# gabrielmpp/LagrangianCoherence

Measured on AMD Instinct MI355X. Metric: particle-timesteps/sec (+ FTLE Mcells/sec) at 4096^2 seeds per GPU, higher is better.
Workload: dtype f32

## Files before the change

### include/lcs_hip.h

```cpp
#ifndef LCS_HIP_H
#define LCS_HIP_H

#include <stddef.h>
#include <stdint.h>

#ifdef __cplusplus
extern "C" {
#endif

#define LC_VERSION 104

typedef struct lc_ctx lc_ctx;

enum lc_dtype {
    LC_F32 = 0,
    LC_F64 = 1,
    LC_F64_WIND_F32 = 2,
    LC_F64_WIND_F32_LIN32 = 3
};

enum lc_status {
    LC_OK = 0,
    LC_EINVAL = -1,
    LC_EUNSUPPORTED = -2,
    LC_EHIP = -3,
    LC_ENOMEM = -4,
    LC_ERCCL = -5
};

enum lc_xboundary {
    LC_X_CLAMP_POINT = 0,
    LC_X_CYCLIC = 1,
    LC_X_CLAMP_REFERENCE_OUTER = 2
};

enum lc_tensor_layout {
    LC_LAYOUT_REFERENCE = 0,
    LC_LAYOUT_PHYSICAL = 1
};

int lc_version(void);
const char *lc_last_error(void);
const char *lc_build_id(void);

int lc_ctx_create(int device, lc_ctx **out);
int lc_ctx_destroy(lc_ctx *ctx);
int lc_ctx_set_stream(lc_ctx *ctx, void *hip_stream );
int lc_ctx_use_own_stream(lc_ctx *ctx);
int lc_sync(lc_ctx *ctx);

int lc_ctx_set_lds_tiles(lc_ctx *ctx, int mode);
int lc_ctx_set_sigma_march(lc_ctx *ctx, int on);
typedef int (*lc_flag_allreduce_fn)(void *user, void *flags_dev, size_t count);
int lc_ctx_set_flag_allreduce(lc_ctx *ctx, lc_flag_allreduce_fn fn, void *user);
int lc_ctx_set_level_chunk(lc_ctx *ctx, int levels);
int lc_ctx_get_level_chunk(const lc_ctx *ctx, int *levels_out);
enum lc_f64_fidelity { LC_F64_AUTO = 0, LC_F64_EXACT_ORDER = 1, LC_F64_FAST = 2 };
#define LC_EXACT_ORDER_MAX_SEEDS (1 << 18)
int lc_ctx_set_f64_fidelity(lc_ctx *ctx, int mode);
int lc_ctx_get_f64_fidelity(const lc_ctx *ctx, int *mode_out);
int lc_ctx_set_host_pipeline(lc_ctx *ctx, int on);
int lc_copy_to_device(lc_ctx *ctx, void *dst_dev, const void *src_host, size_t bytes);
int lc_copy_to_host(lc_ctx *ctx, void *dst_host, const void *src_dev, size_t bytes);
int lc_ctx_set_host_cache(lc_ctx *ctx, int on);
int lc_ctx_trim(lc_ctx *ctx);
int lc_ctx_last_host_marks(const lc_ctx *ctx, double *ms4_out);
int lc_ctx_set_xcd_split(lc_ctx *ctx, int split);
const char *lc_ctx_last_advect_kernel(const lc_ctx *ctx);
int lc_ctx_last_advect_launches(const lc_ctx *ctx);
const char *lc_ctx_last_sigma_kernel(const lc_ctx *ctx);
const char *lc_ctx_last_pack_kernel(const lc_ctx *ctx);
const char *lc_ctx_last_tracer_kernel(const lc_ctx *ctx);
#define LC_VERIFY_WORDS 16
int lc_ctx_set_verify(lc_ctx *ctx, int mode);
int lc_ctx_read_verify(lc_ctx *ctx, unsigned *out16, int reset);

int lc_malloc(lc_ctx *ctx, size_t bytes, void **dev_out);
int lc_free(lc_ctx *ctx, void *dev);
int lc_memcpy_h2d(lc_ctx *ctx, void *dev_dst, const void *host_src, size_t bytes);
int lc_memcpy_d2h(lc_ctx *ctx, void *host_dst, const void *dev_src, size_t bytes);

size_t lc_packed_elems(int nt, int ny_f, int nx_f);
int lc_field_pack(lc_ctx *ctx, const void *u_dev, const void *v_dev, int dtype,
                  int nt, int ny_f, int nx_f, int interp_order, void *packed_dev,
                  void *ext_dev );

int lc_field_extrapolate(lc_ctx *ctx, const void *packed_dev, int dtype,
                         int nt, int ny_f, int nx_f, void *ext_dev);

// ... 153 lines not shown
```

### lagrangiancoherence_amd/_capi.py

```python
from __future__ import annotations

import ctypes as C
import os

HERE = os.path.dirname(os.path.abspath(__file__))
LIB_PATH = os.path.join(HERE, "liblcs_hip.so")

LC_VERSION = 104
LC_F32, LC_F64, LC_F64_WIND_F32, LC_F64_WIND_F32_LIN32 = 0, 1, 2, 3
LC_OK, LC_EINVAL, LC_EUNSUPPORTED, LC_EHIP, LC_ENOMEM, LC_ERCCL = 0, -1, -2, -3, -4, -5
LC_LAYOUT_REFERENCE, LC_LAYOUT_PHYSICAL = 0, 1
LC_X_CLAMP_POINT, LC_X_CYCLIC, LC_X_CLAMP_REFERENCE_OUTER = 0, 1, 2
LC_GRID_REGULAR, LC_GRID_GAUSSIAN = 0, 1
LC_F64_AUTO, LC_F64_EXACT_ORDER, LC_F64_FAST = 0, 1, 2
LC_EXACT_ORDER_MAX_SEEDS = 1 << 18

_vp, _i, _d, _sz = C.c_void_p, C.c_int, C.c_double, C.c_size_t

PROTOTYPES = {
    "lc_version": (_i, []),
    "lc_last_error": (C.c_char_p, []),
    "lc_build_id": (C.c_char_p, []),
    "lc_ctx_create": (_i, [_i, C.POINTER(_vp)]),
    "lc_ctx_destroy": (_i, [_vp]),
    "lc_ctx_set_stream": (_i, [_vp, _vp]),
    "lc_ctx_use_own_stream": (_i, [_vp]),
    "lc_sync": (_i, [_vp]),
    "lc_ctx_set_lds_tiles": (_i, [_vp, _i]),
    "lc_ctx_set_sigma_march": (_i, [_vp, _i]),
    "lc_ctx_set_level_chunk": (_i, [_vp, _i]),
    "lc_ctx_get_level_chunk": (_i, [_vp, C.POINTER(_i)]),
    "lc_ctx_set_f64_fidelity": (_i, [_vp, _i]),
    "lc_ctx_get_f64_fidelity": (_i, [_vp, C.POINTER(_i)]),
    "lc_ctx_set_host_pipeline": (_i, [_vp, _i]),
    "lc_ctx_last_host_marks": (_i, [_vp, C.POINTER(C.c_double)]),
    "lc_copy_to_device": (_i, [_vp, _vp, _vp, C.c_size_t]),
    "lc_copy_to_host": (_i, [_vp, _vp, _vp, C.c_size_t]),
    "lc_ctx_set_host_cache": (_i, [_vp, _i]),
    "lc_ctx_trim": (_i, [_vp]),
    "lc_ctx_set_xcd_split": (_i, [_vp, _i]),
    "lc_ctx_set_flag_allreduce": (_i, [_vp, _vp, _vp]),
    "lc_ctx_last_advect_kernel": (C.c_char_p, [_vp]),
    "lc_ctx_last_advect_launches": (_i, [_vp]),
    "lc_ctx_last_sigma_kernel": (C.c_char_p, [_vp]),
    "lc_ctx_last_pack_kernel": (C.c_char_p, [_vp]),
    "lc_ctx_last_tracer_kernel": (C.c_char_p, [_vp]),
    "lc_ctx_set_verify": (_i, [_vp, _i]),
    "lc_ctx_read_verify": (_i, [_vp, C.POINTER(C.c_uint), _i]),
    "lc_malloc": (_i, [_vp, _sz, C.POINTER(_vp)]),
    "lc_free": (_i, [_vp, _vp]),
    "lc_memcpy_h2d": (_i, [_vp, _vp, _vp, _sz]),
    "lc_memcpy_d2h": (_i, [_vp, _vp, _vp, _sz]),
    "lc_packed_elems": (_sz, [_i, _i, _i]),
    "lc_field_pack": (_i, [_vp, _vp, _vp, _i, _i, _i, _i, _i, _vp, _vp]),
    "lc_field_extrapolate": (_i, [_vp, _vp, _i, _i, _i, _i, _vp]),
    "lc_regrid_common_grid": (_i, [_vp, _vp, _i, _i, _i, _i, _vp, _vp, _vp, _i, _vp, _i, _vp]),
    "lc_spectral_truncate": (_i, [_vp, _vp, _i, _i, _i, _i, _i, _i, _vp]),
    "lc_inspect_gridtype": (_i, [_vp, _i, C.POINTER(_i)]),
    "lc_advect": (_i, [_vp, _vp, _vp, _vp, _i, _i, _i, _i, _d, _d, _d, _d, _vp, _i, _vp, _i, _i, _i,
                       _d, _i, _i, _i, _i, _i, _vp, _vp, _vp, _vp]),
    "lc_advect_from": (_i, [_vp, _vp, _vp, _vp, _i, _i, _i, _i, _d, _d, _d, _d, _vp, _i, _vp, _i, _i, _i, _vp, _vp,
                            _d, _i, _i, _i, _i, _i, _vp, _vp, _vp, _vp]),
    "lc_advect_batch": (_i, [_vp, _vp, _vp, _vp, _i, _i, _i, _i, _d, _d, _d, _d, _vp, _i, _vp, _i, _i, _i, _vp, _vp,
                             _d, _i, _i, _i, _i, _i, _i, _i, _vp, _vp, _vp, _vp]),
# ... 107 lines not shown
```

### lagrangiancoherence_amd/csrc/advect.hip

```cpp
#include <type_traits>
#include <vector>

#include "lcs_common.h"
#include "launch_plan.h"

namespace {

constexpr int TILE_W = 8;
constexpr int TILE_H = 32;
constexpr int BLOCK = TILE_W * TILE_H;

template <typename T>
struct AdvectArgs {
    const T *lin;
    const T *img;
    const T *ext;
    const T *u_raw, *v_raw;
    const float *lin32;
    const float *u_raw32, *v_raw32;
    size_t raw_plane;
    int ext_raw;
    int ext_cub;
    size_t level_elems;
    int pitch;
    int ny_f, nx_f;
    T lat_min, lat_span, lon_min, lon_span;
    T sx, sy;
    T y_min, y_max, x_min, x_max;
    const T *seed_lat, *seed_lon;
    int ny, nx;
    int row0, ny_global;
    T dt, half_dt;
    T dtcy, hdtcy;
    int K, order, cyclic, t0, nsteps;
    int wind_f32;
    T *x_out, *y_out, *traj_x, *traj_y;
    const T *x_start, *y_start;
    int n_members, member_t0_stride;
    size_t member_plane;
    int pair_d, pair_l0, pair_n, pair_g, pair_last;
    size_t pair_plane;
    int traj_skip0;
    int traj_pair_ok, out_pair_ok;
    int traj_line_ok;
    int patch_mode;
    int xcd_rows;
    int xcd_split;
    int wg64;
    int ntx, ntiles;
    int xcd_chunk;
    int tile_order;
    int tile_order_two_seed;
    int pole_blocks, pole_lo, pole_hi;
    unsigned *clamp_flag;
    int clamp_stride;
    unsigned *verify;
    int member_dirs;
};

template <typename T>
__device__ __forceinline__ int xcd_tile_id(const AdvectArgs<T> &A) {
    return lcplan::tile_of_block((int)blockIdx.x - A.pole_blocks, A.ntiles, A.ntx, A.xcd_chunk, A.tile_order);
}
template <typename T>
static inline unsigned nmem(const AdvectArgs<T> &A) { return A.n_members > 1 ? (unsigned)A.n_members : 1u; }

template <typename K, typename T, typename... Extra>
static inline const char *launch_kernel(K kernel, int grid, hipStream_t st, const AdvectArgs<T> &A, const char *name, const Extra &...extra) {
    hipLaunchKernelGGL(kernel, dim3(grid, nmem(A)), dim3(BLOCK), 0, st, A, extra...);
    return name;
}

template <typename T>
struct Pair {
    T u, v;
};

template <typename T>
// ... 1385 lines not shown
            A.traj_y[(size_t)(s + 1) * plane + idx] = p.y;
        }
        lvl += A.level_elems;
        elv += A.level_elems;
    }
    if (live) {
        A.x_out[idx] = p.x;
        A.y_out[idx] = p.y;
    }
}


constexpr int SPL = 2;

#ifndef LCS_LDS2_ROWS
#define LCS_LDS2_ROWS 8
#endif
#ifndef LCS_LDS2_COLS
#define LCS_LDS2_COLS 16
#endif
#ifndef LCS_LDS2_PITCH
#define LCS_LDS2_PITCH (LCS_LDS2_COLS + 4)
#endif
struct Lds2Geom {
    static constexpr int COLS = LCS_LDS2_COLS, LANES_PER_ROW = COLS / 2, ROWS_PER_PASS = 64 / LANES_PER_ROW;
    static_assert(LCS_LDS2_ROWS % ROWS_PER_PASS == 0 || LCS_LDS2_ROWS < ROWS_PER_PASS + 1, "tile rows per staging pass");
};

#ifdef LCS_STAMPS
__device__ unsigned long long g_stamps[8];
__device__ unsigned long long g_cause[4];
__device__ unsigned long long g_redo[3][3][3];
__device__ unsigned long long g_hist[2][5];
#define LCS_STAMP(i)                                           \
    {                                                          \
        const long long _t = __builtin_amdgcn_s_memtime();     \
        acc_t[i] += _t - last_t;                               \
        last_t = _t;                                           \
    }
#else
#define LCS_STAMP(i)
#endif

#ifndef LCS_LDS2_NUM_SGPR
#define LCS_LDS2_NUM_SGPR 96
#endif
constexpr int SLAB_PITCH = 36;

#ifndef LCS_LDS2_MINWAVES
#define LCS_LDS2_MINWAVES 1
#endif
#ifndef LCS_LDS2_DPP_NEXT
#define LCS_LDS2_DPP_NEXT 1
#endif
#ifndef LCS_LDS2_DIRECT_LEVELS
#define LCS_LDS2_DIRECT_LEVELS 0
#endif
template <int KFIX, bool CYCLIC, int MODE>
__global__ void __launch_bounds__(BLOCK, LCS_LDS2_MINWAVES) __attribute__((amdgpu_num_sgpr(LCS_LDS2_NUM_SGPR)))
    advect_lds2_kernel(const AdvectArgs<float> A0) {
#pragma clang fp contract(fast)
    const AdvectArgs<float> A = for_member(A0);
    constexpr bool WIDE = MODE == PATCH_WIDE, LINES = MODE == PATCH_LINES, GROUP = MODE == PATCH_PAIR;
    constexpr int NS = SPL;
    constexpr int ORDER = 1;
    constexpr bool DEFER_X = LCS_LDS2_DEFER_X != 0;
    constexpr int DIRECT_LEVELS = DEFER_X ? LCS_LDS2_DIRECT_LEVELS : 0;
    constexpr bool DPP_NEXT = LCS_LDS2_DPP_NEXT != 0 && 16 % Lds2Geom::LANES_PER_ROW == 0;
    const int K = KFIX >= 0 ? KFIX : A.K;
    typedef Lds2Geom G;
    constexpr int LT_COLS = G::COLS, LT_ROWS = LCS_LDS2_ROWS;
    constexpr int LT_PITCH = LCS_LDS2_PITCH;
    constexpr int WIN = 2, WOFF = LC_PAD_LO;
    __shared__ __attribute__((aligned(16))) f4 s_tiles[BLOCK / 64][LT_ROWS * LT_PITCH];
    __shared__ __attribute__((aligned(16))) float s_slab[2][2][LINES ? 16 * SLAB_PITCH : 4];
    if (GROUP ? pole_block_group(A) : pole_block<float, POLE_LIN>(A)) return;
    const int tile_id = xcd_tile_id(A);
    if (tile_id >= A.ntiles) return;
    const int tyi = tile_id / A.ntx, txi = tile_id - tyi * A.ntx;
    const int lane = threadIdx.x & 63, wave = threadIdx.x >> 6;
    const int ix0 = WIDE ? txi * (TILE_W * SPL) + SPL * (lane % TILE_W)
                  : LINES ? txi * (TILE_W * 4) + wave * TILE_W + (lane % TILE_W) : txi * TILE_W + (lane % TILE_W);
    const int iy0 = (WIDE || GROUP) ? tyi * TILE_H + wave * 8 + lane / TILE_W
                  : LINES ? tyi * (8 * SPL) + lane / TILE_W : tyi * (TILE_H * SPL) + wave * (8 * SPL) + lane / TILE_W;
    f4 *tile = s_tiles[wave];

    bool live[NS];
    f2 p[NS], dd[NS], hd[NS];
    size_t idx[NS];
    const size_t plane = (size_t)A.ny * A.nx;
    bool any = false;
    const int cnt = GROUP ? group_count(A) : NS;
#pragma unroll
    for (int q = 0; q < NS; ++q) {
        const int ix = ix0 + (WIDE ? q : 0), iy = iy0 + ((WIDE || GROUP) ? 0 : 8 * q);
        live[q] = ix < A.nx && iy < A.ny && q < cnt;
        if (live[q]) {
            const int grow = A.row0 + iy;
            if (grow < A.order || grow >= A.ny_global - A.order) {
                if (!A.pole_blocks) {
                    if (GROUP)
                        advect_seed<float, 1, false>(group_member(A, q), A.lin, iy, ix);
                    else
                        advect_seed<float, 1, false>(A, A.lin, iy, ix);
                }
                live[q] = false;
            }
// ... 22 lines not shown
                    dx[off + idx[q]] = p[q].x;
                    dy[off + idx[q]] = p[q].y;
                }
        }
    };
    if (A.traj_x && !A.traj_skip0) store_pair(A.traj_x, A.traj_y, 0);
    const bool lines = LINES && A.traj_x && A.traj_line_ok && (txi + 1) * (TILE_W * 4) <= A.nx;
    if (!lines && __ballot(any) == 0ull) return;
    const int sl_row = (wave & 1) * 8 + (lane >> 3), sl_col = (lane & 7) * 4;
    bool sl_ok = false;
    size_t sl_idx = 0;
    if (lines) {
        const int iyr = tyi * (8 * SPL) + sl_row, grow = A.row0 + iyr;
        sl_ok = iyr < A.ny && (A.pole_blocks == 0 || (grow >= A.order && grow < A.ny_global - A.order));
        if (!A.pole_blocks && iyr < A.ny && (grow < A.order || grow >= A.ny_global - A.order)) sl_ok = false;
        sl_idx = (size_t)min(iyr, A.ny - 1) * A.nx + (size_t)txi * (TILE_W * 4) + sl_col;
    }
    float ymax_v = A.y_max;
    asm volatile("" : "+v"(ymax_v));
    const unsigned tile_addr = lds_address(tile);
    unsigned pitch_bytes = (unsigned)LT_PITCH * 16u;
    asm volatile("" : "+s"(pitch_bytes));
    const f2 pmin = {A.lon_min, A.lat_min}, sc = {A.sx, A.sy};
    auto to_index = [&](f2 v) { return (v - pmin) * sc; };
    const float xlo = A.x_min, xhi = A.x_max;
    auto x_needs_care = [&](float x) { return CYCLIC ? !(fabsf(x) < 180.0f) : !((x > xlo) & (x < xhi)); };
    const float *lvl = A.img + (size_t)A.t0 * A.level_elems;
    const float *elv = A.ext + (size_t)A.t0 * A.level_elems;
    const int pad_cols = A.pitch, pad_rows = A.ny_f + LC_PAD;
    const float kpred = 0.5f * (float)(K > 0 ? K - 1 : 0);
    const int st_row = min(lane / G::LANES_PER_ROW, LT_ROWS - 1), st_col = (lane % G::LANES_PER_ROW) * 2;
    const unsigned st_off = ((unsigned)st_row * (unsigned)pad_cols + (unsigned)st_col) * 8u;
    constexpr int NPASS = (LT_ROWS + G::ROWS_PER_PASS - 1) / G::ROWS_PER_PASS;
    const unsigned st_next = st_off + (st_col + 2 < LT_COLS ? 16u : 0u);
    constexpr int CENTRE = (WIDE || GROUP) ? TILE_W / 2 + TILE_W * 4 : TILE_W / 2 + TILE_W * 7;
    f2 dprev = {0.0f, 0.0f};
    const int nlev = GROUP ? lcplan::group_levels(A.nsteps, A.pair_l0, A.pair_n, A.pair_d, cnt) : A.nsteps;
#ifdef LCS_STAMPS
    long long acc_t[5] = {0, 0, 0, 0, 0}, last_t = __builtin_amdgcn_s_memtime();
    unsigned long long acc_n[3] = {0, 0, 0};
    int prev_redos = 0;
#endif
    int direct_left = 0;
    for (int s = 0; s < nlev; ++s) {
        const bool direct = DIRECT_LEVELS > 0 && direct_left > 0;
        if (direct) --direct_left;
#ifdef LCS_STAMPS
        int level_redos = 0;
#endif
        f2 c0[NS];
#pragma unroll
        for (int q = 0; q < NS; ++q) c0[q] = to_index(p[q]);
        bool act[NS];
        f2 keep[NS];
        int qa = 0;
        if (GROUP) {
            int qlo = NS, qhi = 0;
#pragma unroll
            for (int q = 0; q < NS; ++q) {
                act[q] = lcplan::member_steps(q, s, A.pair_l0, A.pair_n, A.pair_d) && q < cnt;
                keep[q] = p[q];
                if (act[q]) {
                    qlo = min(qlo, q);
                    qhi = q;
                }
            }
            qa = min(max(NS / 2, qlo), qhi);
        }
        auto of_anchor = [&](const f2 (&v)[NS]) {
            f2 r = v[0];
#pragma unroll
            for (int q = 1; q < NS; ++q) r = (GROUP && qa == q) ? v[q] : r;
            return r;
        };
        int ox = 0, oy = 0;
        f4 stage[NPASS];
        f2 stage_next[NPASS];
        if (K > 0 && !direct) {
            const f2 ca = dprev * (1.0f + kpred) + of_anchor(c0);
            const int rxm = __builtin_amdgcn_readlane((int)floor_to_uint(ca.x), CENTRE);
            const int rym = __builtin_amdgcn_readlane((int)floor_to_uint(ca.y), CENTRE);
            ox = min(max(rxm + WOFF - (LT_COLS - WIN) / 2, 0), pad_cols - LT_COLS);
            oy = min(max(rym + WOFF - (LT_ROWS - WIN) / 2, 0), pad_rows - LT_ROWS);
            const char *src = (const char *)elv + ((size_t)__umul24((unsigned)oy, (unsigned)pad_cols) + (unsigned)ox) * 8;
#pragma unroll
            for (int r = 0; r < NPASS; ++r) {
                __builtin_memcpy(&stage[r], src + (size_t)(r * G::ROWS_PER_PASS) * pad_cols * 8 + st_off, 16);
                if (!DPP_NEXT) __builtin_memcpy(&stage_next[r], src + (size_t)(r * G::ROWS_PER_PASS) * pad_cols * 8 + st_next, 8);
            }
        }
        LCS_STAMP(0)
        f2 e[NS], pn[NS];
        bool bad[NS], anybad = false;
#pragma unroll
        for (int q = 0; q < NS; ++q) {
            const TapL t = tap_of(c0[q]);
            bad[q] = ((unsigned)t.x0 > (unsigned)(A.nx_f - 2)) | ((unsigned)t.y0 > (unsigned)(A.ny_f - 2));
            e[q] = euler_global<ORDER>(lvl, A, t);
            pn[q] = dd[q] * e[q] + p[q];
            if (!DEFER_X) bad[q] |= x_needs_care(pn[q].x);
            anybad |= bad[q];
        }
        if (anybad) {
#pragma unroll
            for (int q = 0; q < NS; ++q) {
                if (bad[q]) {
                    const TapL t = tap_of(index_coords(A, p[q]));
                    e[q] = euler_global<ORDER>(lvl, A, t);
                    pn[q] = dd[q] * e[q] + p[q];
                    if (!DEFER_X) clamp_position_p(A, pn[q], ymax_v);
                }
            }
        }
        dprev = (of_anchor(pn) - of_anchor(p)) * sc;
#pragma unroll
        for (int q = 0; q < NS; ++q) p[q] = pn[q];
#ifdef LCS_STAMPS
        asm volatile("" : : "v"(p[0].x), "v"(p[1].x));
#endif
        LCS_STAMP(1)
        int lo_x = 0x40000000, lo_y = 0x40000000, lim_x = 0, lim_y = 0;
        unsigned base_addr = tile_addr;
        if (K > 0 && !direct) {
            __builtin_amdgcn_wave_barrier();
#pragma unroll
            for (int r = 0; r < NPASS; ++r) {
                f2 nxt;
                if constexpr (DPP_NEXT) {
                    float nx0, nx1;
                    const float s0 = stage[r].x, s1 = stage[r].y;
                    asm volatile("s_nop 4\n\tv_mov_b32_dpp %0, %2 row_shl:1 row_mask:0xf bank_mask:0xf bound_ctrl:0\n\t"
                                 "v_mov_b32_dpp %1, %3 row_shl:1 row_mask:0xf bank_mask:0xf bound_ctrl:0"
                                 : "=&v"(nx0), "=&v"(nx1) : "v"(s0), "v"(s1));
                    nxt = (f2){nx0, nx1};
                } else {
                    nxt = stage_next[r];
                }
                f4 *dst = tile + (r * G::ROWS_PER_PASS + st_row) * LT_PITCH + st_col;
                const f2 n0 = stage[r].xy, n1 = stage[r].zw, d0 = n1 - n0, d1 = nxt - n1;
                dst[0] = (f4){n0.x, n0.y, d0.x, d0.y};
                dst[1] = (f4){n1.x, n1.y, d1.x, d1.y};
            }
            __builtin_amdgcn_wave_barrier();
            const int sox = ox - WOFF, soy = oy - WOFF;
            const int hx = min(sox + LT_COLS - WIN, A.nx_f - 2), hy = min(soy + LT_ROWS - WIN, A.ny_f - 2);
            const int lx = max(sox, DEFER_X ? 1 : 0), ly = max(soy, DEFER_X ? 1 : 0);
            if (hx >= lx && hy >= ly) {
                lo_x = lx;
                lo_y = ly;
                lim_x = hx - lx;
                lim_y = hy - ly;
                base_addr = tile_addr + (unsigned)(lx - sox) * 16u + (unsigned)(ly - soy) * ((unsigned)LT_PITCH * 16u);
            }
        }
#ifdef LCS_STAMPS
        asm volatile("s_waitcnt vmcnt(0) lgkmcnt(0)" ::: "memory");
#endif
        LCS_STAMP(2)
        int redos = 0;
        if (direct) {
#pragma unroll 1
            for (int k = 0; k < K; ++k) {
#pragma unroll
                for (int q = 0; q < NS; ++q) {
                    f2 pc = p[q];
                    clamp_position_c<CYCLIC>(A, pc, ymax_v);
                    const TapL t = tap_of(index_coords(A, pc));
                    p[q] = hd[q] * window_global<ORDER>(elv, A, t, e[q]) + pc;
                }
            }
        } else
#pragma unroll
        for (int k = 0; k < K; ++k) {
            anybad = false;
#pragma unroll
            for (int q = 0; q < NS; ++q) {
                typedef __attribute__((address_space(3))) const f4 lds_f4;
                const TapL t = tap_of(to_index(p[q]));
                const int rx = t.x0 - lo_x, ry = t.y0 - lo_y;
                bad[q] = ((unsigned)rx > (unsigned)lim_x) | ((unsigned)ry > (unsigned)lim_y);
#ifdef LCS_STAMPS
                {
                    const unsigned long long bx = __ballot((unsigned)rx > (unsigned)lim_x), by = __ballot((unsigned)ry > (unsigned)lim_y);
                    const unsigned long long bxl = __ballot(rx < 0), byl = __ballot(ry < 0);
                    if (lane == 0) {
                        atomicAdd(&g_cause[0], (unsigned long long)__popcll(bx));
                        atomicAdd(&g_cause[1], (unsigned long long)__popcll(by));
                        atomicAdd(&g_cause[2], (unsigned long long)__popcll(bxl));
                        atomicAdd(&g_cause[3], (unsigned long long)__popcll(byl));
                    }
                }
#endif
                unsigned row_addr;
                asm("v_mad_u32_u24 %0, %1, %2, %3" : "=v"(row_addr) : "v"(ry), "s"(pitch_bytes), "v"(base_addr));
                lds_f4 *cell = (lds_f4 *)(size_t)(row_addr + ((unsigned)rx << 4));
                const f4 c0 = cell[0], c1 = cell[LT_PITCH];
                const f2 r0 = c0.xy + t.tx * c0.zw;
                const f2 r1 = c1.xy + t.tx * c1.zw;
                const f2 ew = e[q] + (r0 + t.ty * (r1 - r0));
                pn[q] = hd[q] * ew + p[q];
                if (!DEFER_X) bad[q] |= x_needs_care(pn[q].x);
                anybad |= bad[q];
            }
#ifdef LCS_STAMPS
            {
                const unsigned long long m0 = __ballot(bad[0]), m1 = __ballot(bad[1]);
                if (lane == 0) {
                    acc_n[0] += 1;
                    acc_n[1] += (m0 | m1) ? 1 : 0;
                    level_redos += (m0 | m1) ? 1 : 0;
                    acc_n[2] += __popcll(m0) + __popcll(m1);
                    const int band = min(2, (int)(fabsf(A.seed_lat[min(iy0, A.ny - 1)]) / 30.0f)), third = min(2, 3 * s / A.nsteps);
                    atomicAdd(&g_redo[band][third][0], 1ull);
                    atomicAdd(&g_redo[band][third][1], (m0 | m1) ? 1ull : 0ull);
                    atomicAdd(&g_redo[band][third][2], (unsigned long long)(__popcll(m0) + __popcll(m1)));
                }
            }
#endif
            if (DIRECT_LEVELS > 0) redos += __ballot(anybad) != 0ull;
            if (anybad) {
#pragma unroll
                for (int q = 0; q < NS; ++q) {
                    if (bad[q]) {
                        f2 pc = p[q];
                        if (DEFER_X)
                            clamp_position_c<CYCLIC>(A, pc, ymax_v);
                        else
                            pc.y = __builtin_amdgcn_fmed3f(pc.y, A.y_min, ymax_v);
                        const TapL t = tap_of(index_coords(A, pc));
                        pn[q] = hd[q] * window_global<ORDER>(elv, A, t, e[q]) + pc;
                        if (!DEFER_X) clamp_position_p(A, pn[q], ymax_v);
                    }
                }
            }
#pragma unroll
            for (int q = 0; q < NS; ++q) p[q] = pn[q];
        }
        if (DIRECT_LEVELS > 0 && redos >= 3) direct_left = DIRECT_LEVELS;
#pragma unroll
        for (int q = 0; q < NS; ++q) {
            if (DEFER_X)
                clamp_position_c<CYCLIC>(A, p[q], ymax_v);
            else
                p[q].y = __builtin_amdgcn_fmed3f(p[q].y, A.y_min, ymax_v);
        }
        if (GROUP) {
#pragma unroll
            for (int q = 0; q < NS; ++q)
                if (!act[q]) p[q] = keep[q];
        }
        if (LINES && lines) {
            float *sx = s_slab[s & 1][0], *sy = s_slab[s & 1][1];
#pragma unroll
            for (int q = 0; q < NS; ++q) {
                const int o = (lane / TILE_W + 8 * q) * SLAB_PITCH + wave * TILE_W + (lane % TILE_W);
                sx[o] = p[q].x;
                sy[o] = p[q].y;
            }
            asm volatile("s_waitcnt lgkmcnt(0)\n\ts_barrier" ::: "memory");
            const f4 line = *(const f4 *)(s_slab[s & 1][wave >> 1] + sl_row * SLAB_PITCH + sl_col);
            if (sl_ok) {
                float *dst = ((wave >> 1) ? A.traj_y : A.traj_x) + (size_t)(s + 1) * plane + sl_idx;
                LCS_TRAJ_STORE(dst, line);
            }
        } else if (A.traj_x) {
            store_pair(A.traj_x, A.traj_y, (size_t)(s + 1) * plane);
        }
#ifdef LCS_STAMPS
        asm volatile("" : : "v"(p[0].x), "v"(p[1].x));
#endif
        LCS_STAMP(3)
// ... 1759 lines not shown
    A.order = g.interp_order;
}

struct AdvectCall {
    FieldSource src;
    const void *ext;
    const void *lin32, *lin32_v;
    int wind_f32;
    bool series;
    int dirs;
};

template <typename T>
int advect_impl(lc_ctx *ctx, const lc_advect_args &a, const AdvectCall &call) {
    const int ny = a.ny, nx = a.nx, order = a.interp_order, K = a.settls_order, t0_stride = a.t0_stride;
    const int n_members = a.n_members * call.dirs;
    AdvectArgs<T> A{};
    A.member_dirs = call.dirs == 2;
    A.wind_f32 = call.wind_f32;
    A.n_members = n_members;
    A.member_t0_stride = t0_stride;
    A.member_plane = (size_t)ny * nx;
    A.x_start = (const T *)a.x_start;
    A.y_start = (const T *)a.y_start;
    A.traj_skip0 = 0;
    A.pair_d = -1;
    A.traj_pair_ok = (nx % 2 == 0) && ((size_t)a.traj_x % (2 * sizeof(T)) == 0) && ((size_t)a.traj_y % (2 * sizeof(T)) == 0);
    A.out_pair_ok = (nx % 2 == 0) && ((size_t)a.x_out % (2 * sizeof(T)) == 0) && ((size_t)a.y_out % (2 * sizeof(T)) == 0);
    A.traj_line_ok = (nx % 4 == 0) && ((size_t)a.traj_x % 16 == 0) && ((size_t)a.traj_y % 16 == 0) && sizeof(T) == 4;
    A.patch_mode = ctx->patch_mode;
    A.xcd_rows = ctx->xcd_chunk_rows;
    A.xcd_split = ctx->xcd_split;
    set_field_geometry(A, call.src, a);
    A.ext = (order == 1 || order == 3) ? (const T *)call.ext : nullptr;
    A.lin32 = (sizeof(T) == 8 && order == 1) ? (const float *)call.lin32 : nullptr;
    A.u_raw32 = (sizeof(T) == 8 && order == 3) ? (const float *)call.lin32 : nullptr;
    A.v_raw32 = (sizeof(T) == 8 && order == 3) ? (const float *)call.lin32_v : nullptr;
    A.ext_raw = a.fuse_levels_raw && sizeof(T) == 8 && order == 1 && call.src.u_raw && !call.wind_f32 && !call.ext;
    A.ext_cub = a.fuse_levels_raw && sizeof(T) == 8 && order == 3 && call.src.cub && !call.wind_f32 && !call.ext;
    A.y_min = (T)a.lat_min;
    A.y_max = (T)a.lat_max;
    A.x_min = (T)a.lon_min;
    A.x_max = (T)a.lon_max;
    A.seed_lat = (const T *)a.seed_lat_dev;
    A.seed_lon = (const T *)a.seed_lon_dev;
    const double conv_y = 180.0 / (6371000.0 * 3.141592653589793);
    A.dt = (T)a.timestep;
    A.half_dt = (T)(0.5 * a.timestep);
    A.dtcy = (T)(a.timestep * conv_y);
    A.hdtcy = (T)((0.5 * a.timestep) * conv_y);
    A.K = K;
    const bool outer = a.cyclic_x == LC_X_CLAMP_REFERENCE_OUTER;
    A.cyclic = a.cyclic_x == LC_X_CYCLIC;
    A.clamp_flag = nullptr;
    A.verify = sizeof(T) == 4 ? ctx->verify_dev : nullptr;
    unsigned *clamp_flag = nullptr;
    const bool per_member = outer && call.series && n_members > 1;
    const int n_flags = per_member ? n_members : 1;
    if (outer) {
        LC_HIP_CHECK(hipMallocAsync((void **)&clamp_flag, n_flags * sizeof(unsigned), ctx->stream));
        (void)hipMemsetAsync(clamp_flag, 0, n_flags * sizeof(unsigned), ctx->stream);
        A.clamp_flag = clamp_flag;
        A.clamp_stride = per_member ? 1 : 0;
    }
    A.t0 = a.t0;
    A.nsteps = a.nsteps;
// ... 345 lines not shown
        {"tracer_kernel<double, 1>", "tracer_kernel<double, 2>", "tracer_kernel<double, 3>", "tracer_kernel<double, 4>", "tracer_kernel<double, 5>"}};
#define LC_TRACER(ORD)                                                                                                  \
    hipLaunchKernelGGL((tracer_kernel<T, ORD>), dim3(blocks), dim3(256), 0, ctx->stream, A, (const T *)a.traj_x,          \
                       (const T *)a.traj_y, a.level0, a.n_levels, O)
    switch (a.interp_order) {
        case 2: LC_TRACER(2); break;
        case 3: LC_TRACER(3); break;
        case 4: LC_TRACER(4); break;
        case 5: LC_TRACER(5); break;
        default: LC_TRACER(1); break;
    }
#undef LC_TRACER
    LC_HIP_CHECK(hipGetLastError());
    ctx->last_tracer_kernel = names[sizeof(T) == 8][a.interp_order - 1];
    return LC_OK;
}

}

#ifdef LCS_STAMPS
extern "C" int lc_debug_read_cause(unsigned long long *out4, int reset) {
    if (hipMemcpyFromSymbol(out4, HIP_SYMBOL(g_cause), sizeof(g_cause)) != hipSuccess) return -1;
    if (reset) {
        unsigned long long z[4] = {};
        if (hipMemcpyToSymbol(HIP_SYMBOL(g_cause), z, sizeof(z)) != hipSuccess) return -1;
    }
    return 0;
}
extern "C" int lc_debug_read_hist(unsigned long long *out10, int reset) {
    if (hipMemcpyFromSymbol(out10, HIP_SYMBOL(g_hist), sizeof(g_hist)) != hipSuccess) return -1;
    if (reset) {
        unsigned long long z[10] = {};
        if (hipMemcpyToSymbol(HIP_SYMBOL(g_hist), z, sizeof(z)) != hipSuccess) return -1;
    }
    return 0;
}
extern "C" int lc_debug_read_redo(unsigned long long *out27, int reset) {
    if (hipMemcpyFromSymbol(out27, HIP_SYMBOL(g_redo), sizeof(g_redo)) != hipSuccess) return -1;
    if (reset) {
        unsigned long long z[27] = {};
        if (hipMemcpyToSymbol(HIP_SYMBOL(g_redo), z, sizeof(z)) != hipSuccess) return -1;
    }
    return 0;
}
extern "C" int lc_debug_read_stamps(unsigned long long *out8, int reset) {
    if (hipMemcpyFromSymbol(out8, HIP_SYMBOL(g_stamps), sizeof(g_stamps)) != hipSuccess) return -1;
    if (reset) {
        unsigned long long z[8] = {};
        if (hipMemcpyToSymbol(HIP_SYMBOL(g_stamps), z, sizeof(z)) != hipSuccess) return -1;
    }
    return 0;
}
#endif

static bool raw_replaces_lin(const void *u_raw, const void *v_raw, int dtype, int interp_order) {
    return u_raw && v_raw && (interp_order != 1 || dtype != LC_F32);
}

extern "C" int lc_sample_raw(lc_ctx *ctx, const void *packed_lin, const void *packed_cub, const void *u_raw, const void *v_raw,
                             int dtype, int nt, int ny_f, int nx_f, double lat_min, double lat_max, double lon_min,
                             double lon_max, int level, const void *pos_x_dev, const void *pos_y_dev, int ny, int nx, int row0,
                             int ny_global, int interp_order, void *out_u, void *out_v) {
    LC_REQUIRE(ctx, "lc_sample: null context");
    LC_REQUIRE(dtype == LC_F32 || dtype == LC_F64, "lc_sample: bad dtype %d", dtype);
    if (interp_order < 1 || interp_order > 5) {
        lc_set_error("lc_sample: interp_order %d unsupported (scipy's spline orders 1..5; 0 fails in the reference)", interp_order);
// ... 238 lines not shown
```

### lagrangiancoherence_amd/csrc/api.hip

```cpp
#include <chrono>
#include <cmath>
#include <cstdlib>
#include <cstring>
#include <vector>

#include "hostxfer.h"
#include "lcs_common.h"

static thread_local char g_err[1024] = "";

void lc_set_error(const char *fmt, ...) {
    va_list ap;
    va_start(ap, fmt);
    vsnprintf(g_err, sizeof(g_err), fmt, ap);
    va_end(ap);
}

extern "C" const char *lc_last_error(void) { return g_err; }
extern "C" int lc_version(void) { return LC_VERSION; }
#ifndef LCS_BUILD_ID
#define LCS_BUILD_ID "unstamped"
#endif
extern "C" const char *lc_build_id(void) { return LCS_BUILD_ID; }

// ... 16 lines not shown
        lc_set_error("hipStreamCreate failed: %s", hipGetErrorString(e));
        delete c;
        return LC_EHIP;
    }
    c->stream = c->own_stream;
    c->n_cus = 256;
    {
        int n = 0;
        if (hipDeviceGetAttribute(&n, hipDeviceAttributeMultiprocessorCount, c->device) == hipSuccess && n > 0) c->n_cus = n;
        else (void)hipGetLastError();
    }
    c->lds_tiles = 3;
    if (const char *ev = getenv("LCS_LDS_TILES")) c->lds_tiles = ev[0] == '0' ? 0 : (ev[0] == '2' ? 2 : (ev[0] == '1' ? 1 : 3));
    c->xcd_chunk_rows = 1;
    if (const char *ev = getenv("LCS_XCD_CHUNK_ROWS")) c->xcd_chunk_rows = atoi(ev) > 0 ? atoi(ev) : 0;
    c->xcd_split = -1;
    if (const char *ev = getenv("LCS_XCD_SPLIT")) c->xcd_split = atoi(ev) >= 0 ? atoi(ev) : -1;
    c->tile_order = -1;
    if (const char *ev = getenv("LCS_TILE_ORDER")) c->tile_order = (ev[0] >= '0' && ev[0] <= '3') ? ev[0] - '0' : -1;
    c->pole_blocks = 1;
    if (const char *ev = getenv("LCS_POLE_BLOCKS")) c->pole_blocks = ev[0] != '0';
    c->fir_prefilter = 1;
    if (const char *ev = getenv("LCS_FIR_PREFILTER")) c->fir_prefilter = ev[0] == '0' ? 0 : (ev[0] == '2' ? 2 : 1);
    c->fused_prefilter = 1;
    if (const char *ev = getenv("LCS_FUSED_PREFILTER")) c->fused_prefilter = ev[0] != '0';
    c->sigma_march = 2;
    if (const char *ev = getenv("LCS_SIGMA_MARCH")) c->sigma_march = ev[0] == '0' ? 0 : (ev[0] == '1' ? 1 : 2);
    c->level_chunk = -1;
    if (const char *ev = getenv("LCS_LEVEL_CHUNK")) c->level_chunk = atoi(ev) >= 0 ? atoi(ev) : -1;
    c->f64_fidelity = LC_F64_AUTO;
    if (const char *ev = getenv("LCS_F64_FIDELITY")) c->f64_fidelity = ev[0] == 'e' ? LC_F64_EXACT_ORDER : (ev[0] == 'f' ? LC_F64_FAST : LC_F64_AUTO);
    c->patch_mode = -1;
    if (const char *ev = getenv("LCS_PATCH_MODE")) c->patch_mode = (ev[0] >= '0' && ev[0] <= '3') ? ev[0] - '0' : -1;
    c->flag_reduce = nullptr;
    c->flag_reduce_user = nullptr;
    c->lds_tiles_init = c->lds_tiles;
    c->sigma_march_init = c->sigma_march;
    c->last_advect_kernel = "";
    c->last_advect_launches = 0;
    c->last_sigma_kernel = "";
    c->last_pack_kernel = "";
    c->last_tracer_kernel = "";
    c->last_strain_kernel = "";
    c->verify_dev = nullptr;
    c->trunc = nullptr;
    c->xfer = nullptr;
    c->host_ws = nullptr;
    c->host_cache = 1;
    if (const char *ev = getenv("LCS_HOST_CACHE")) c->host_cache = ev[0] != '0';
    c->host_timing = getenv("LCS_HOST_TIMING") != nullptr;
    for (double &m : c->host_marks) m = 0.0;
    c->host_pipeline = 1;
    if (const char *ev = getenv("LCS_HOST_PIPELINE")) c->host_pipeline = ev[0] != '0';
    c->f64_wg_tile = 0;
    if (const char *ev = getenv("LCS_F64_WG_TILE")) c->f64_wg_tile = ev[0] == '1';
    c->host_threads = -1;
    c->host_piece_mb = 0;
    if (const char *ev = getenv("LCS_HOST_THREADS")) c->host_threads = atoi(ev);
    if (const char *ev = getenv("LCS_HOST_PIECE_MB")) c->host_piece_mb = std::min(std::max(atoi(ev), 1), 256);
    *out = c;
    return LC_OK;
}

extern "C" int lc_ctx_set_lds_tiles(lc_ctx *ctx, int mode) {
    LC_REQUIRE(ctx, "lc_ctx_set_lds_tiles: null context");
    LC_REQUIRE(mode >= -1 && mode <= 2, "lc_ctx_set_lds_tiles: mode must be -1, 0, 1 or 2");
// ... 75 lines not shown
    a.row0 = 0;
    a.ny_global = ny;
    a.timestep = timestep;
    a.settls_order = K;
    a.interp_order = order;
    a.cyclic_x = cyclic_x;
    a.t0 = t0;
    a.nsteps = nsteps;
    a.n_members = 1;
    a.t0_stride = 0;
    a.x_out = x;
    a.y_out = y;
    a.traj_x = tx;
    a.traj_y = ty;
    return lc_advect_ex(ctx, &a);
}

static bool f64_exact_order(const lc_ctx *ctx, int dtype, int ny, int nx) {
    if (dtype != LC_F64) return false;
    return ctx->f64_fidelity == LC_F64_EXACT_ORDER ||
           (ctx->f64_fidelity == LC_F64_AUTO && (long long)ny * nx <= LC_EXACT_ORDER_MAX_SEEDS);
}

extern "C" int lc_ctx_get_level_chunk(const lc_ctx *ctx, int *levels_out) {
    LC_REQUIRE(ctx && levels_out, "lc_ctx_get_level_chunk: null pointer");
    *levels_out = ctx->level_chunk;
    return LC_OK;
}

extern "C" int lc_ctx_set_level_chunk(lc_ctx *ctx, int levels) {
    LC_REQUIRE(ctx, "lc_ctx_set_level_chunk: null context");
    LC_REQUIRE(levels >= -1, "lc_ctx_set_level_chunk: levels must be >= -1 (0 = one launch for the whole series, -1 = by size)");
    ctx->level_chunk = levels;
    return LC_OK;
}

extern "C" int lc_ctx_set_verify(lc_ctx *ctx, int mode) {
    LC_REQUIRE(ctx, "lc_ctx_set_verify: null context");
    LC_REQUIRE(mode >= 0 && mode <= 2, "lc_ctx_set_verify: mode must be 0 (off), 1 (audit) or 2 (audit + one injected corruption)");
    LC_HIP_CHECK(hipSetDevice(ctx->device));
    LC_HIP_CHECK(hipStreamSynchronize(ctx->stream));
    if (mode == 0) {
        if (ctx->verify_dev) LC_HIP_CHECK(hipFree(ctx->verify_dev));
        ctx->verify_dev = nullptr;
        return LC_OK;
    }
    if (!ctx->verify_dev) {
        hipError_t e = hipMalloc((void **)&ctx->verify_dev, LC_VERIFY_WORDS * sizeof(unsigned));
        if (e != hipSuccess) {
            ctx->verify_dev = nullptr;
            (void)hipGetLastError();
            lc_set_error("lc_ctx_set_verify: hipMalloc failed: %s", hipGetErrorString(e));
            return e == hipErrorOutOfMemory ? LC_ENOMEM : LC_EHIP;
        }
    }
    unsigned init[LC_VERIFY_WORDS] = {};
    init[15] = mode == 2 ? 0xBADu : 0u;
    LC_HIP_CHECK(hipMemcpy(ctx->verify_dev, init, sizeof(init), hipMemcpyHostToDevice));
    return LC_OK;
}

extern "C" int lc_ctx_read_verify(lc_ctx *ctx, unsigned *out16, int reset) {
    LC_REQUIRE(ctx && out16, "lc_ctx_read_verify: null pointer");
    LC_REQUIRE(ctx->verify_dev, "lc_ctx_read_verify: the audit is off (lc_ctx_set_verify)");
    LC_HIP_CHECK(hipSetDevice(ctx->device));
    LC_HIP_CHECK(hipStreamSynchronize(ctx->stream));
// ... 744 lines not shown
```

### lagrangiancoherence_amd/csrc/lcs_common.h

```cpp
#pragma once
#include <hip/hip_runtime.h>

#include <cstdarg>
#include <cstdio>

#include "../../include/lcs_hip.h"

struct lc_trunc_cache;
void lc_trunc_cache_free(lc_trunc_cache *c);

struct lc_ctx {
    int device;
    int n_cus;
    hipStream_t own_stream;
    hipStream_t stream;
    int lds_tiles;
    int lds_tiles_init, sigma_march_init;
    int sigma_march;
    int xcd_split;
    int xcd_chunk_rows;
    int fir_prefilter;
    int fused_prefilter;
    int tile_order;
    int pole_blocks;
    int level_chunk;
    int f64_fidelity;
    int patch_mode;
    lc_flag_allreduce_fn flag_reduce;
    void *flag_reduce_user;
    int last_advect_launches;
    const char *last_advect_kernel;
    const char *last_sigma_kernel;
    const char *last_pack_kernel;
    const char *last_tracer_kernel;
    unsigned *verify_dev;
    lc_trunc_cache *trunc;
    struct lc_host_xfer *xfer;
    void *host_ws;
    int host_cache;
    double host_marks[4];
    int host_timing;
    int f64_wg_tile;
    int host_threads;
    int host_piece_mb;
    int host_pipeline;
    const char *last_strain_kernel;
};

void lc_set_error(const char *fmt, ...);

#define LC_HIP_CHECK(expr)                                                              \
    do {                                                                                \
        hipError_t _e = (expr);                                                         \
        if (_e != hipSuccess) {                                                         \
            lc_set_error("%s failed: %s (%s:%d)", #expr, hipGetErrorString(_e), __FILE__, \
                         __LINE__);                                                     \
            (void)hipGetLastError();                                                    \
            return LC_EHIP;                                                             \
        }                                                                               \
    } while (0)

#define LC_REQUIRE(cond, ...)          \
    do {                               \
        if (!(cond)) {                 \
            lc_set_error(__VA_ARGS__); \
            return LC_EINVAL;          \
        }                              \
    } while (0)

constexpr int LC_PAD_LO = 1;
constexpr int LC_PAD_HI = 2;
constexpr int LC_PAD = LC_PAD_LO + LC_PAD_HI;

static inline size_t lc_level_elems(int ny_f, int nx_f) {
    return (size_t)(ny_f + LC_PAD) * (size_t)(nx_f + LC_PAD) * 2;
}

int lc_launch_pack(lc_ctx *ctx, const void *u, const void *v, int dtype, int nt, int ny_f, int nx_f,
                   int order, void *packed, void *ext);
int lc_launch_extrapolate(lc_ctx *ctx, const void *img, int dtype, int nt, int ny_f, int nx_f, void *ext);
// ... 1 lines not shown
```

### lagrangiancoherence_amd/engine.py

```python
from __future__ import annotations

import ctypes as C
import os
from dataclasses import dataclass

import numpy as np

from . import _capi

__all__ = ["Engine", "PackedField", "PackedTracer", "lcs_host", "lcs_global_host", "common_dtype", "x_boundary_mode"]

_NP2LC = {np.dtype(np.float32): _capi.LC_F32, np.dtype(np.float64): _capi.LC_F64}
_LAYOUTS = {"reference": _capi.LC_LAYOUT_REFERENCE, "physical": _capi.LC_LAYOUT_PHYSICAL}


def x_boundary_mode(cyclic_xboundary, noncyclic_clamp=None, whole_grid=True) -> int:
    if cyclic_xboundary:
        return _capi.LC_X_CYCLIC
    if noncyclic_clamp is None:
        noncyclic_clamp = "reference_outer"
    if noncyclic_clamp not in ("pointwise", "reference_outer"):
        raise ValueError(f"noncyclic_clamp {noncyclic_clamp!r}: 'pointwise' or 'reference_outer'")
    return _capi.LC_X_CLAMP_REFERENCE_OUTER if noncyclic_clamp == "reference_outer" else _capi.LC_X_CLAMP_POINT

# ... 61 lines not shown
        _capi.check(self.lib.lc_ctx_create(self.device_index, C.byref(ctx)), self.lib)
        self.lds_tiles_mode = -1
        self.verify_mode = 0
        self._poison = bool(os.environ.get("LCS_DEBUG_POISON"))
        self.ctx = ctx

    def close(self):
        if getattr(self, "ctx", None):
            self.lib.lc_ctx_destroy(self.ctx)
            self.ctx = None

    def __del__(self):
        try:
            self.close()
        except Exception:
            pass

    def set_lds_tiles(self, mode: int):
        _capi.check(self.lib.lc_ctx_set_lds_tiles(self.ctx, int(mode)), self.lib)
        self.lds_tiles_mode = int(mode)

    def set_sigma_march(self, on: int):
        _capi.check(self.lib.lc_ctx_set_sigma_march(self.ctx, int(on)), self.lib)

    def set_level_chunk(self, levels: int):
        _capi.check(self.lib.lc_ctx_set_level_chunk(self.ctx, int(levels)), self.lib)

    @property
    def level_chunk(self) -> int:
        v = C.c_int()
        _capi.check(self.lib.lc_ctx_get_level_chunk(self.ctx, C.byref(v)), self.lib)
        return v.value

    _FIDELITY = {"auto": _capi.LC_F64_AUTO, "exact": _capi.LC_F64_EXACT_ORDER, "fast": _capi.LC_F64_FAST}

    def set_f64_fidelity(self, mode: str):
        if mode not in self._FIDELITY:
            raise ValueError(f"float64 fidelity {mode!r}: 'auto', 'exact' or 'fast'")
        _capi.check(self.lib.lc_ctx_set_f64_fidelity(self.ctx, self._FIDELITY[mode]), self.lib)

    def f64_fuse_levels(self, dtype, n_seeds: int) -> bool:
        if np.dtype(dtype) != np.dtype(np.float64):
            return True
        m = C.c_int()
        _capi.check(self.lib.lc_ctx_get_f64_fidelity(self.ctx, C.byref(m)), self.lib)
        if m.value == _capi.LC_F64_EXACT_ORDER:
            return False
        return m.value == _capi.LC_F64_FAST or int(n_seeds) > _capi.LC_EXACT_ORDER_MAX_SEEDS

    def set_flag_allreduce(self, group=None, comm=None, enable=True):
        if not enable:
            _capi.check(self.lib.lc_ctx_set_flag_allreduce(self.ctx, None, None), self.lib)
            self._flag_cb = None
            return
        if comm is not None:
            fn = C.cast(self.lib.lc_comm_flag_allreduce, C.c_void_p)
            _capi.check(self.lib.lc_ctx_set_flag_allreduce(self.ctx, fn, comm), self.lib)
            self._flag_cb = None
            return
        torch = self.torch
        import torch.distributed as dist

        class _DeviceWords:
            def __init__(self, ptr, n):
                self.__cuda_array_interface__ = {"shape": (int(n),), "typestr": "<i4", "data": (int(ptr), False), "version": 2}

        def reduce(_user, ptr, count):
            try:
                t = torch.as_tensor(_DeviceWords(ptr, count), device=self.device)
                if dist.get_backend(group) == "gloo":
                    h = t.cpu()
                    dist.all_reduce(h, op=dist.ReduceOp.MAX, group=group)
                    t.copy_(h)
                else:
                    dist.all_reduce(t, op=dist.ReduceOp.MAX, group=group)
                return 0
            except Exception:
                import traceback
                traceback.print_exc()
                return 1
        self._flag_cb = _capi.FLAG_ALLREDUCE_FN(reduce)
        _capi.check(self.lib.lc_ctx_set_flag_allreduce(self.ctx, C.cast(self._flag_cb, C.c_void_p), None), self.lib)

    def last_advect_kernel(self) -> str:
        return self.lib.lc_ctx_last_advect_kernel(self.ctx).decode()

    def set_verify(self, mode: int = 1):
        _capi.check(self.lib.lc_ctx_set_verify(self.ctx, int(mode)), self.lib)
        self.verify_mode = int(mode)

    def read_verify(self, reset: bool = True) -> dict:
        out = (C.c_uint * 16)()
        _capi.check(self.lib.lc_ctx_read_verify(self.ctx, out, int(bool(reset))), self.lib)
        v = [int(x) for x in out]
        d = {"tile_changed": v[0], "entries_changed": v[1], "slot_changes": v[2], "audited": v[3]}
        if v[12]:
            d["first_event"] = {"workgroup": v[4], "tile": v[5], "wave": v[6], "level": v[7], "hw_id_before": hex(v[8]),
                                "hw_id_after": hex(v[9]), "lane_mask": hex(v[10] | (v[11] << 32))}
        return d

    def last_advect_launches(self) -> int:
        return int(self.lib.lc_ctx_last_advect_launches(self.ctx))

    TWO_SEED_MIN = 1 << 23
    EXT_IMAGE_F64 = True
    EXT_IMAGE_F64_O3 = True

    class _Concurrent:

        def __init__(self, eng, seeds_per_call, n):
            self.eng, self.force = eng, eng.lds_tiles_mode == -1 and "LCS_LDS_TILES" not in os.environ \
                and seeds_per_call < Engine.TWO_SEED_MIN <= seeds_per_call * n

        def __enter__(self):
            if self.force:
                self.eng.set_lds_tiles(1)
            return self

        def __exit__(self, *exc):
            if self.force:
                self.eng.set_lds_tiles(-1)
            return False

    def concurrent_calls(self, seeds_per_call: int, n: int):
        return Engine._Concurrent(self, int(seeds_per_call), int(n))

    def last_sigma_kernel(self) -> str:
        return self.lib.lc_ctx_last_sigma_kernel(self.ctx).decode()
# ... 875 lines not shown
```

Baseline: 250.3 billion.

## Adaptively grow the LDS2 staged tile height after repeated out-of-tile redos

Adds an adaptive mode to the LDS2 advection kernel. When a wave's particles leave the staged field window too often within a level, the kernel stages a taller tile (16 rows) for the next several levels to cut the cost of redoing out-of-window taps. The mode is gated by a context flag that defaults off (LCS_LDS2_GROW=0). Even when it is off, the kernel now reserves shared memory for the larger tile, carries bigger stage arrays and computes ballots every substep to count redos, which may lower occupancy and add instruction overhead.

```diff
diff --git a/include/lcs_hip.h b/include/lcs_hip.h
--- a/include/lcs_hip.h
+++ b/include/lcs_hip.h
@@ -55,6 +55,7 @@
 int lc_ctx_set_flag_allreduce(lc_ctx *ctx, lc_flag_allreduce_fn fn, void *user);
 int lc_ctx_set_level_chunk(lc_ctx *ctx, int levels);
 int lc_ctx_get_level_chunk(const lc_ctx *ctx, int *levels_out);
+int lc_ctx_set_lds2_grow(lc_ctx *ctx, int on);
 enum lc_f64_fidelity { LC_F64_AUTO = 0, LC_F64_EXACT_ORDER = 1, LC_F64_FAST = 2 };
 #define LC_EXACT_ORDER_MAX_SEEDS (1 << 18)
 int lc_ctx_set_f64_fidelity(lc_ctx *ctx, int mode);
diff --git a/lagrangiancoherence_amd/_capi.py b/lagrangiancoherence_amd/_capi.py
--- a/lagrangiancoherence_amd/_capi.py
+++ b/lagrangiancoherence_amd/_capi.py
@@ -30,6 +30,7 @@
     "lc_ctx_set_sigma_march": (_i, [_vp, _i]),
     "lc_ctx_set_level_chunk": (_i, [_vp, _i]),
     "lc_ctx_get_level_chunk": (_i, [_vp, C.POINTER(_i)]),
+    "lc_ctx_set_lds2_grow": (_i, [_vp, _i]),
     "lc_ctx_set_f64_fidelity": (_i, [_vp, _i]),
     "lc_ctx_get_f64_fidelity": (_i, [_vp, C.POINTER(_i)]),
     "lc_ctx_set_host_pipeline": (_i, [_vp, _i]),
diff --git a/lagrangiancoherence_amd/csrc/advect.hip b/lagrangiancoherence_amd/csrc/advect.hip
--- a/lagrangiancoherence_amd/csrc/advect.hip
+++ b/lagrangiancoherence_amd/csrc/advect.hip
@@ -44,6 +44,7 @@
     int traj_pair_ok, out_pair_ok;
     int traj_line_ok;
     int patch_mode;
+    int lds2_grow;
     int xcd_rows;
     int xcd_split;
     int wg64;
@@ -1495,6 +1496,7 @@
 __device__ unsigned long long g_cause[4];
 __device__ unsigned long long g_redo[3][3][3];
 __device__ unsigned long long g_hist[2][5];
+__device__ unsigned long long g_grown;
 #define LCS_STAMP(i)                                           \
     {                                                          \
         const long long _t = __builtin_amdgcn_s_memtime();     \
@@ -1518,6 +1520,12 @@
 #endif
 #ifndef LCS_LDS2_DIRECT_LEVELS
 #define LCS_LDS2_DIRECT_LEVELS 0
+#endif
+#ifndef LCS_LDS2_GROWN_ROWS
+#define LCS_LDS2_GROWN_ROWS 16
+#endif
+#ifndef LCS_LDS2_GROW_LEVELS
+#define LCS_LDS2_GROW_LEVELS 7
 #endif
 template <int KFIX, bool CYCLIC, int MODE>
 __global__ void __launch_bounds__(BLOCK, LCS_LDS2_MINWAVES) __attribute__((amdgpu_num_sgpr(LCS_LDS2_NUM_SGPR)))
@@ -1535,7 +1543,12 @@
     constexpr int LT_COLS = G::COLS, LT_ROWS = LCS_LDS2_ROWS;
     constexpr int LT_PITCH = LCS_LDS2_PITCH;
     constexpr int WIN = 2, WOFF = LC_PAD_LO;
-    __shared__ __attribute__((aligned(16))) f4 s_tiles[BLOCK / 64][LT_ROWS * LT_PITCH];
+    constexpr int GROWN_ROWS = LCS_LDS2_GROWN_ROWS;
+    constexpr bool CAN_GROW = KFIX != 0 && DIRECT_LEVELS == 0 && LT_ROWS == G::ROWS_PER_PASS && GROWN_ROWS > LT_ROWS &&
+                              GROWN_ROWS % G::ROWS_PER_PASS == 0;
+    constexpr int MAX_ROWS = CAN_GROW ? GROWN_ROWS : LT_ROWS;
+    constexpr bool COUNT_REDOS = DIRECT_LEVELS > 0 || CAN_GROW;
+    __shared__ __attribute__((aligned(16))) f4 s_tiles[BLOCK / 64][MAX_ROWS * LT_PITCH];
     __shared__ __attribute__((aligned(16))) float s_slab[2][2][LINES ? 16 * SLAB_PITCH : 4];
     if (GROUP ? pole_block_group(A) : pole_block<float, POLE_LIN>(A)) return;
     const int tile_id = xcd_tile_id(A);
@@ -1624,6 +1637,7 @@
     const int st_row = min(lane / G::LANES_PER_ROW, LT_ROWS - 1), st_col = (lane % G::LANES_PER_ROW) * 2;
     const unsigned st_off = ((unsigned)st_row * (unsigned)pad_cols + (unsigned)st_col) * 8u;
     constexpr int NPASS = (LT_ROWS + G::ROWS_PER_PASS - 1) / G::ROWS_PER_PASS;
+    constexpr int NPASS_MAX = (MAX_ROWS + G::ROWS_PER_PASS - 1) / G::ROWS_PER_PASS;
     const unsigned st_next = st_off + (st_col + 2 < LT_COLS ? 16u : 0u);
     constexpr int CENTRE = (WIDE || GROUP) ? TILE_W / 2 + TILE_W * 4 : TILE_W / 2 + TILE_W * 7;
     f2 dprev = {0.0f, 0.0f};
@@ -1634,9 +1648,13 @@
     int prev_redos = 0;
 #endif
     int direct_left = 0;
+    int grow_left = 0;
+    const int grow_trigger = (CAN_GROW && A.lds2_grow) ? min(K, 3) : 0x7fffffff;
     for (int s = 0; s < nlev; ++s) {
         const bool direct = DIRECT_LEVELS > 0 && direct_left > 0;
         if (direct) --direct_left;
+        const bool grown = CAN_GROW && grow_left > 0;
+        const int rows = grown ? GROWN_ROWS : LT_ROWS;
 #ifdef LCS_STAMPS
         int level_redos = 0;
 #endif
@@ -1666,19 +1684,21 @@
             return r;
         };
         int ox = 0, oy = 0;
-        f4 stage[NPASS];
-        f2 stage_next[NPASS];
+        f4 stage[NPASS_MAX];
+        f2 stage_next[NPASS_MAX];
         if (K > 0 && !direct) {
             const f2 ca = dprev * (1.0f + kpred) + of_anchor(c0);
             const int rxm = __builtin_amdgcn_readlane((int)floor_to_uint(ca.x), CENTRE);
             const int rym = __builtin_amdgcn_readlane((int)floor_to_uint(ca.y), CENTRE);
             ox = min(max(rxm + WOFF - (LT_COLS - WIN) / 2, 0), pad_cols - LT_COLS);
-            oy = min(max(rym + WOFF - (LT_ROWS - WIN) / 2, 0), pad_rows - LT_ROWS);
+            oy = min(max(rym + WOFF - (rows - WIN) / 2, 0), pad_rows - rows);
             const char *src = (const char *)elv + ((size_t)__umul24((unsigned)oy, (unsigned)pad_cols) + (unsigned)ox) * 8;
 #pragma unroll
-            for (int r = 0; r < NPASS; ++r) {
-                __builtin_memcpy(&stage[r], src + (size_t)(r * G::ROWS_PER_PASS) * pad_cols * 8 + st_off, 16);
-                if (!DPP_NEXT) __builtin_memcpy(&stage_next[r], src + (size_t)(r * G::ROWS_PER_PASS) * pad_cols * 8 + st_next, 8);
+            for (int r = 0; r < NPASS_MAX; ++r) {
+                if (r < NPASS || grown) {
+                    __builtin_memcpy(&stage[r], src + (size_t)(r * G::ROWS_PER_PASS) * pad_cols * 8 + st_off, 16);
+                    if (!DPP_NEXT) __builtin_memcpy(&stage_next[r], src + (size_t)(r * G::ROWS_PER_PASS) * pad_cols * 8 + st_next, 8);
+                }
             }
         }
         LCS_STAMP(0)
@@ -1716,7 +1736,8 @@
         if (K > 0 && !direct) {
             __builtin_amdgcn_wave_barrier();
 #pragma unroll
-            for (int r = 0; r < NPASS; ++r) {
+            for (int r = 0; r < NPASS_MAX; ++r) {
+                if (r >= NPASS && !grown) continue;
                 f2 nxt;
                 if constexpr (DPP_NEXT) {
                     float nx0, nx1;
@@ -1734,8 +1755,14 @@
                 dst[1] = (f4){n1.x, n1.y, d1.x, d1.y};
             }
             __builtin_amdgcn_wave_barrier();
+            if (CAN_GROW && grown) {
+                if (A.verify && lane == 0) atomicAdd(&A.verify[13], 1u);
+#ifdef LCS_STAMPS
+                if (lane == 0) atomicAdd(&g_grown, 1ull);
+#endif
+            }
             const int sox = ox - WOFF, soy = oy - WOFF;
-            const int hx = min(sox + LT_COLS - WIN, A.nx_f - 2), hy = min(soy + LT_ROWS - WIN, A.ny_f - 2);
+            const int hx = min(sox + LT_COLS - WIN, A.nx_f - 2), hy = min(soy + rows - WIN, A.ny_f - 2);
             const int lx = max(sox, DEFER_X ? 1 : 0), ly = max(soy, DEFER_X ? 1 : 0);
             if (hx >= lx && hy >= ly) {
                 lo_x = lx;
@@ -1765,12 +1792,14 @@
 #pragma unroll
         for (int k = 0; k < K; ++k) {
             anybad = false;
+            unsigned long long left = 0ull;
 #pragma unroll
             for (int q = 0; q < NS; ++q) {
                 typedef __attribute__((address_space(3))) const f4 lds_f4;
                 const TapL t = tap_of(to_index(p[q]));
                 const int rx = t.x0 - lo_x, ry = t.y0 - lo_y;
                 bad[q] = ((unsigned)rx > (unsigned)lim_x) | ((unsigned)ry > (unsigned)lim_y);
+                if (COUNT_REDOS) left |= __builtin_amdgcn_ballot_w64((unsigned)rx > (unsigned)lim_x) | __builtin_amdgcn_ballot_w64((unsigned)ry > (unsigned)lim_y);
 #ifdef LCS_STAMPS
                 {
                     const unsigned long long bx = __ballot((unsigned)rx > (unsigned)lim_x), by = __ballot((unsigned)ry > (unsigned)lim_y);
@@ -1792,6 +1821,7 @@
                 const f2 ew = e[q] + (r0 + t.ty * (r1 - r0));
                 pn[q] = hd[q] * ew + p[q];
                 if (!DEFER_X) bad[q] |= x_needs_care(pn[q].x);
+                if (!DEFER_X && COUNT_REDOS) left |= __builtin_amdgcn_ballot_w64(x_needs_care(pn[q].x));
                 anybad |= bad[q];
             }
 #ifdef LCS_STAMPS
@@ -1809,7 +1839,10 @@
                 }
             }
 #endif
-            if (DIRECT_LEVELS > 0) redos += __ballot(anybad) != 0ull;
+            if (COUNT_REDOS) {
+                redos = __builtin_amdgcn_readfirstlane(redos + (left != 0ull));
+                asm volatile("" : "+s"(redos));
+            }
             if (anybad) {
 #pragma unroll
                 for (int q = 0; q < NS; ++q) {
@@ -1829,6 +1862,12 @@
             for (int q = 0; q < NS; ++q) p[q] = pn[q];
         }
         if (DIRECT_LEVELS > 0 && redos >= 3) direct_left = DIRECT_LEVELS;
+        if (CAN_GROW) {
+            if (grown)
+                --grow_left;
+            else if (redos >= grow_trigger)
+                grow_left = LCS_LDS2_GROW_LEVELS;
+        }
 #pragma unroll
         for (int q = 0; q < NS; ++q) {
             if (DEFER_X)
@@ -3654,6 +3693,7 @@
     A.xcd_rows = ctx->xcd_chunk_rows;
     A.xcd_split = ctx->xcd_split;
     set_field_geometry(A, call.src, a);
+    A.lds2_grow = ctx->lds2_grow && A.ny_f + LC_PAD >= LCS_LDS2_GROWN_ROWS;
     A.ext = (order == 1 || order == 3) ? (const T *)call.ext : nullptr;
     A.lin32 = (sizeof(T) == 8 && order == 1) ? (const float *)call.lin32 : nullptr;
     A.u_raw32 = (sizeof(T) == 8 && order == 3) ? (const float *)call.lin32 : nullptr;
@@ -4065,6 +4105,14 @@
     if (reset) {
         unsigned long long z[10] = {};
         if (hipMemcpyToSymbol(HIP_SYMBOL(g_hist), z, sizeof(z)) != hipSuccess) return -1;
+    }
+    return 0;
+}
+extern "C" int lc_debug_read_grown(unsigned long long *out1, int reset) {
+    if (hipMemcpyFromSymbol(out1, HIP_SYMBOL(g_grown), sizeof(g_grown)) != hipSuccess) return -1;
+    if (reset) {
+        unsigned long long z = 0;
+        if (hipMemcpyToSymbol(HIP_SYMBOL(g_grown), &z, sizeof(z)) != hipSuccess) return -1;
     }
     return 0;
 }
diff --git a/lagrangiancoherence_amd/csrc/api.hip b/lagrangiancoherence_amd/csrc/api.hip
--- a/lagrangiancoherence_amd/csrc/api.hip
+++ b/lagrangiancoherence_amd/csrc/api.hip
@@ -72,6 +72,7 @@
     if (const char *ev = getenv("LCS_F64_FIDELITY")) c->f64_fidelity = ev[0] == 'e' ? LC_F64_EXACT_ORDER : (ev[0] == 'f' ? LC_F64_FAST : LC_F64_AUTO);
     c->patch_mode = -1;
     if (const char *ev = getenv("LCS_PATCH_MODE")) c->patch_mode = (ev[0] >= '0' && ev[0] <= '3') ? ev[0] - '0' : -1;
+    c->lds2_grow = LCS_LDS2_GROW != 0;
     c->flag_reduce = nullptr;
     c->flag_reduce_user = nullptr;
     c->lds_tiles_init = c->lds_tiles;
@@ -213,6 +214,13 @@
     LC_REQUIRE(ctx, "lc_ctx_set_level_chunk: null context");
     LC_REQUIRE(levels >= -1, "lc_ctx_set_level_chunk: levels must be >= -1 (0 = one launch for the whole series, -1 = by size)");
     ctx->level_chunk = levels;
+    return LC_OK;
+}
+
+extern "C" int lc_ctx_set_lds2_grow(lc_ctx *ctx, int on) {
+    LC_REQUIRE(ctx, "lc_ctx_set_lds2_grow: null context");
+    LC_REQUIRE(on >= -1 && on <= 1, "lc_ctx_set_lds2_grow: on must be 1, 0 or -1 (the library's default)");
+    ctx->lds2_grow = on < 0 ? LCS_LDS2_GROW != 0 : on;
     return LC_OK;
 }
 
diff --git a/lagrangiancoherence_amd/csrc/lcs_common.h b/lagrangiancoherence_amd/csrc/lcs_common.h
--- a/lagrangiancoherence_amd/csrc/lcs_common.h
+++ b/lagrangiancoherence_amd/csrc/lcs_common.h
@@ -26,6 +26,7 @@
     int level_chunk;
     int f64_fidelity;
     int patch_mode;
+    int lds2_grow;
     lc_flag_allreduce_fn flag_reduce;
     void *flag_reduce_user;
     int last_advect_launches;
@@ -46,6 +47,10 @@
     int host_pipeline;
     const char *last_strain_kernel;
 };
+
+#ifndef LCS_LDS2_GROW
+#define LCS_LDS2_GROW 0
+#endif
 
 void lc_set_error(const char *fmt, ...);
 
diff --git a/lagrangiancoherence_amd/engine.py b/lagrangiancoherence_amd/engine.py
--- a/lagrangiancoherence_amd/engine.py
+++ b/lagrangiancoherence_amd/engine.py
@@ -117,6 +117,9 @@
         _capi.check(self.lib.lc_ctx_get_level_chunk(self.ctx, C.byref(v)), self.lib)
         return v.value
 
+    def set_lds2_grow(self, on: int):
+        _capi.check(self.lib.lc_ctx_set_lds2_grow(self.ctx, int(on)), self.lib)
+
     _FIDELITY = {"auto": _capi.LC_F64_AUTO, "exact": _capi.LC_F64_EXACT_ORDER, "fast": _capi.LC_F64_FAST}
 
     def set_f64_fidelity(self, mode: str):
@@ -178,7 +181,7 @@
         out = (C.c_uint * 16)()
         _capi.check(self.lib.lc_ctx_read_verify(self.ctx, out, int(bool(reset))), self.lib)
         v = [int(x) for x in out]
-        d = {"tile_changed": v[0], "entries_changed": v[1], "slot_changes": v[2], "audited": v[3]}
+        d = {"tile_changed": v[0], "entries_changed": v[1], "slot_changes": v[2], "audited": v[3], "grown_levels": v[13]}
         if v[12]:
             d["first_event"] = {"workgroup": v[4], "tile": v[5], "wave": v[6], "level": v[7], "hw_id_before": hex(v[8]),
                                 "hw_id_after": hex(v[9]), "lane_mask": hex(v[10] | (v[11] << 32))}
```

Result: slower. 240.5 billion (-3.9%).
